# arnauqb/GradABM-JUNE

Hardware: AMD Instinct MI355X
Metric: simulation steps/sec (higher is better)
Workload: dtype f32

## Files before the change

### gradabm-june_amd/csrc/gj_tiled.h

```cpp
#pragma once
#include <hip/hip_runtime.h>
#include <stdint.h>

#include <type_traits>

#include "../../include/gradjune_hip.h"
#include "gj_device.h"

namespace gj {

constexpr int kTileThreads = 1024;
constexpr int kTileWaves = kTileThreads / kWave;
constexpr int kMaxSliceAgents = 19840;
constexpr int kUnroll = 8;
#ifndef GJ_UNROLL_NARROW
#define GJ_UNROLL_NARROW 16
#endif
constexpr int kUnrollNarrow = GJ_UNROLL_NARROW;
#ifndef GJ_VENUE_UNROLL
#define GJ_VENUE_UNROLL 2
#endif
constexpr int kVenueUnroll = GJ_VENUE_UNROLL;
#ifndef GJ_VENUE_UNROLL_C
#define GJ_VENUE_UNROLL_C GJ_VENUE_UNROLL
// ... 418 lines not shown
  const float* v_pc;
  float* cum;
  int32_t stride;
  int32_t nk;
  float beta[GJ_MAX_NETS_PER_SET];
  int32_t table[GJ_MAX_NETS_PER_SET];
  int32_t age75[GJ_MAX_NETS_PER_SET];
  int32_t leisure;
  int32_t direct;
  uint32_t term_limit;
  int32_t _pad_b;
  const uint16_t* pv_blk;
  const int32_t* blk_r0;
  const float* x;
  int64_t n_x;
};

struct TileBArgs {
  TSetB sets[GJ_MAX_SETS];
  const int32_t* work;
  const float* tables;
  int32_t day_type;
  int32_t mode;
  int32_t transpose;
  int32_t _pad;
};

struct ClassWeights {
  float l, lw;
};
__device__ __forceinline__ ClassWeights class_weights(const float* tables, int table, int age75, int day_type, int c) {
// ... 183 lines not shown
#pragma unroll
    for (int u = 0; u < kVenueUnroll; ++u) {
      const int gu = g + u * kTileThreads;
      if (gu >= gb) continue;
      Group8 G(raw[u], make_uint2(0u, 0u), xa[u], xb[u]);
#pragma unroll
      for (int q = 0; q < 8; ++q) {
        const int a = gu * 8 + q;
        if (!(a >= r0 && a < r1)) G.drop(q);
      }
      run_sums(W, G, 0, sums, vflags);
    }
  }
}

__device__ __forceinline__ void venue_cum_write(const VenueItem& W, const fx_t* sums, const uint32_t* vflags, float* cumf) {
  const TSetB& T = W.T;
  for (int l0 = W.tid; l0 < W.nv; l0 += kCumBatch * kTileThreads) {
    float pc[kCumBatch];
#pragma unroll
    for (int u = 0; u < kCumBatch; ++u) pc[u] = T.v_pc[W.v0 + min(l0 + u * kTileThreads, W.nv - 1)];
    for (int k = 0; k < W.nk; ++k) {
      const float beta = T.beta[k];
#pragma unroll
      for (int u = 0; u < kCumBatch; ++u) {
        const int lv = l0 + u * kTileThreads;
        if (lv < W.nv) {
          const float c = (beta * pc[u]) * fx_read<kFxVenue>(sums, vflags, W.vwords, k * W.nv + lv);
          T.cum[(int64_t)(W.v0 + lv) * T.stride + k] = c;
          cumf[2 * (k * W.nv + lv)] = c;
// ... 59 lines not shown
      store_nt(W.val4() + 2 * gu + 1, make_float4(r[4], r[5], r[6], r[7]));
    }
  }
}

#ifndef GJ_VENUE_WAVES_PER_SIMD
#define GJ_VENUE_WAVES_PER_SIMD 4
#endif
__global__ __launch_bounds__(kTileThreads, GJ_VENUE_WAVES_PER_SIMD) void k_tile_venues(const TileBArgs B) {
  extern __shared__ __align__(16) float lds_s[];
  [[maybe_unused]] const VenueStamp gj_stamp;
  const int set = B.work[2 * blockIdx.x], j = B.work[2 * blockIdx.x + 1];
  const TSetB& T = B.sets[set];
  if (T.nk == 0) return;
  const VenueItem W(T, j, lds_s, threadIdx.x);
  if (T.leisure) fill_class_weights<true, true>(W.tabs, W.tabs + W.nk * 200, T, B.tables, B.day_type, B.transpose, W.tid);
  if (B.mode != 2) {
    venue_zero(W, W.sums, W.vflags);
    __syncthreads();
    venue_sums_tiled(W, W.tabs, W.sums, W.vflags);
    if (T.pv_blk) venue_sums_runs(W, j, W.sums, W.vflags);
    __syncthreads();
    venue_cum_write(W, W.sums, W.vflags, W.cumf);
    if (B.mode == 1 || T.direct) return;
  } else {
    if (T.direct) return;
    venue_cum_read(W, W.cumf);
  }
  __syncthreads();
  venue_gather(W, W.tabs + W.nk * 200, W.cumf);
}

constexpr int GJ_MAX_PRESUM = 6;
constexpr int64_t kPresumBad = (int64_t)0x8000000000000000ll;
struct TPSet {
  const uint16_t* ell;
  int64_t plane_stride;
  fx_t* partial;
  int32_t planes, V, stride, nk;
  int32_t group_venues;
  int32_t raw, leisure, _pad;
  int32_t table[GJ_MAX_NETS_PER_SET];
  int32_t age75[GJ_MAX_NETS_PER_SET];
};
struct TilePArgs {
  TPSet sets[GJ_MAX_PRESUM];
  int32_t n_sets;
  int32_t agents_per_wg;
  int64_t n_agents;
  const float* trans;
  const float* qtrans;
  const uint8_t* cls;
  const float* tables;
  int32_t day_type, transpose;
};

constexpr int kPresumQuads = 3;
__device__ __forceinline__ void fx_add_or_poison(fx_t* sums, uint32_t* flags, int i, float x) {
  const bool ok = fabsf(x) <= fx_max<kFxVenue>();
  atomicAdd(&sums[i], to_fx<kFxVenue>(ok ? x : 0.0f));
  if (__builtin_expect(!ok, 0)) atomicOr(&flags[i >> 5], 1u << (i & 31));
}

__global__ __launch_bounds__(kTileThreads) void k_tile_presum(const TilePArgs P) {
  extern __shared__ __align__(16) fx_t lds_p[];
  const int tid = threadIdx.x;
  const int64_t a_begin = (int64_t)blockIdx.x * P.agents_per_wg;
  const int64_t a_end = min(P.n_agents, a_begin + P.agents_per_wg);
  const int n_quads = (int)((max(a_end - a_begin, (int64_t)0) + 3) >> 2);
  for (int t = 0; t < P.n_sets; ++t) {
    const TPSet& T = P.sets[t];
    const int nk = T.nk;
    const float* x = T.raw ? P.trans : P.qtrans;
    for (int v0 = 0; v0 < T.V; v0 += T.group_venues) {
      const int nv = min(T.group_venues, T.V - v0);
      const int n_sums = nv * nk;
      const int dummy = n_sums + (tid & 63);
      float* wtab = reinterpret_cast<float*>(lds_p + n_sums + 64);
      uint32_t* flags = reinterpret_cast<uint32_t*>(wtab + (T.leisure ? nk * 200 : 0));
      __syncthreads();
      for (int i = tid; i < n_sums + 64; i += kTileThreads) lds_p[i] = 0;
      for (int i = tid; i < (n_sums + 64 + 31) / 32; i += kTileThreads) flags[i] = 0u;
      if (T.leisure) fill_class_weights<true, false>(wtab, nullptr, T, P.tables, P.day_type, P.transpose, tid);
      __syncthreads();
      for (int plane = 0; plane < T.planes; ++plane) {
        const uint16_t* ell = T.ell + plane * T.plane_stride + a_begin * 2;
        struct Batch {
          uint4 rows[kPresumQuads];
          float4 xs[kPresumQuads];
          uint32_t cl[kPresumQuads];
        };
        auto load = [&](int b0, Batch& B) {
#pragma unroll
          for (int u = 0; u < kPresumQuads; ++u) {
            const int q = min(b0 + tid + u * kTileThreads, n_quads - 1);
            const int64_t a0 = a_begin + 4 * (int64_t)q;
            B.rows[u] = *reinterpret_cast<const uint4*>(ell + 8 * (int64_t)q);
            if (a0 + 4 <= P.n_agents) {
              B.xs[u] = *reinterpret_cast<const float4*>(x + a0);
            } else {
              B.xs[u] = make_float4(a0 < P.n_agents ? x[a0] : 0.0f, a0 + 1 < P.n_agents ? x[a0 + 1] : 0.0f,
                                    a0 + 2 < P.n_agents ? x[a0 + 2] : 0.0f, 0.0f);
            }
            B.cl[u] = T.leisure ? *reinterpret_cast<const uint32_t*>(P.cls + a0) : 0u;
          }
        };
        auto add = [&](int b0, const Batch& B) {
#pragma unroll
          for (int u = 0; u < kPresumQuads; ++u) {
            const int q = b0 + tid + u * kTileThreads;
            if (q >= n_quads) continue;
            const uint32_t w[4] = {B.rows[u].x, B.rows[u].y, B.rows[u].z, B.rows[u].w};
            const float xv[4] = {B.xs[u].x, B.xs[u].y, B.xs[u].z, B.xs[u].w};
            const int n_ok = (int)min((int64_t)4, a_end - (a_begin + 4 * (int64_t)q));
#pragma unroll
            for (int j = 0; j < 4; ++j) {
#pragma unroll
              for (int c = 0; c < 2; ++c) {
                const int lv = (int)((w[j] >> (16 * c)) & 0xFFFF) - v0;
                const bool in = ((unsigned)lv < (unsigned)nv) && (j < n_ok);
                if (!T.leisure) {
                  fx_add_or_poison(lds_p, flags, in ? lv : dummy, in ? xv[j] : 0.0f);
                } else {
                  const int cj = class_byte(B.cl[u], j);
                  for (int k = 0; k < nk; ++k)
                    fx_add_or_poison(lds_p, flags, in ? lv * nk + k : dummy, in ? wtab[k * 200 + cj] * xv[j] : 0.0f);
                }
              }
            }
          }
        };
        constexpr int kStep = kPresumQuads * kTileThreads;
        if (n_quads > 0) {
          Batch ba, bb;
          int b0 = 0;
          load(b0, ba);
          while (true) {
            const bool more1 = b0 + kStep < n_quads;
            if (more1) load(b0 + kStep, bb);
            add(b0, ba);
            if (!more1) break;
            b0 += kStep;
            const bool more2 = b0 + kStep < n_quads;
            if (more2) load(b0 + kStep, ba);
            add(b0, bb);
            if (!more2) break;
            b0 += kStep;
          }
        }
      }
      __syncthreads();
      fx_t* out = T.partial + (int64_t)blockIdx.x * T.V * T.stride;
      for (int i = tid; i < n_sums; i += kTileThreads) {
        const int lv = i / nk, k = i % nk;
        const bool bad = (flags[i >> 5] >> (i & 31)) & 1u;
        out[(int64_t)(v0 + lv) * T.stride + k] = bad ? (fx_t)kPresumBad : lds_p[i];
      }
    }
  }
}

struct PReduceSet {
  const fx_t* partial;
  const float* v_pc;
  float* cum;
  int32_t V, stride, nk, first;
  float beta[GJ_MAX_NETS_PER_SET];
};
struct PReduceArgs {
  PReduceSet sets[GJ_MAX_PRESUM];
  int32_t n_sets, n_wgs;
  int32_t total;
  int32_t _pad;
};

__global__ __launch_bounds__(kThreads) void k_presum_reduce(const PReduceArgs R) {
  __shared__ fx_t part[kThreads / kWave][kWave];
  __shared__ uint32_t bad_any[kWave];
  const int lane = threadIdx.x % kWave, wave = threadIdx.x / kWave;
  const int i = blockIdx.x * kWave + lane;
  const bool in = i < R.total;
  int t = 0;
  while (t + 1 < R.n_sets && i >= R.sets[t + 1].first) ++t;
  const PReduceSet& T = R.sets[t];
  const int e = in ? i - T.first : 0;
  const int v = e / T.nk, k = e % T.nk;
  const int64_t idx = (int64_t)v * T.stride + k, table = (int64_t)T.V * T.stride;
  fx_t s = 0;
  bool bad = false;
  if (threadIdx.x < kWave) bad_any[threadIdx.x] = 0u;
  constexpr int kWaves = kThreads / kWave;
  for (int w0 = wave; w0 < R.n_wgs; w0 += kWaves * 8) {
    fx_t p[8];
#pragma unroll
    for (int u = 0; u < 8; ++u) {
      const int w = w0 + u * kWaves;
      p[u] = (in && w < R.n_wgs) ? T.partial[w * table + idx] : (fx_t)0;
    }
#pragma unroll
    for (int u = 0; u < 8; ++u) {
      bad |= p[u] == (fx_t)kPresumBad;
      s += p[u];
    }
  }
  part[wave][lane] = s;
  __syncthreads();
  if (bad) atomicOr(&bad_any[lane], 1u);
  __syncthreads();
  if (wave == 0 && in) {
    fx_t total = 0;
#pragma unroll
    for (int w = 0; w < kWaves; ++w) total += part[w][lane];
    T.cum[idx] = (T.beta[k] * T.v_pc[v]) * (bad_any[lane] ? __builtin_nanf("") : from_fx<kFxVenue>(total));
  }
}

constexpr int GJ_MAX_DIRECT = GJ_MAX_SETS;
constexpr int kClassWeightFloats = GJ_MAX_NETS_PER_SET * 200;
struct TDirect {
  const uint16_t* ell;
  const float* cum;
  int64_t plane_stride;
  int32_t planes;
  int32_t V, stride, nk;
  int32_t region;
  int32_t group_venues;
  int32_t raw, leisure;
  int32_t table[GJ_MAX_NETS_PER_SET];
// ... 518 lines not shown
```

### gradabm-june_amd/csrc/gradjune_hip.hip

```cpp
#include <hip/hip_runtime.h>
#include <math.h>
#include <stdint.h>
#include <string.h>

#include "../../include/gradjune_hip.h"
#include "gj_device.h"
#include "gj_tiled.h"
#include "gj_agent.h"
#include "gj_location.h"

namespace gj {

struct SetP1 {
  const int32_t* v_rowptr;
  const int32_t* v_agent;
  const float* v_pc;
  float* cum;
  int32_t stride;
  int32_t nk;
  float beta[GJ_MAX_NETS_PER_SET];
  int32_t table[GJ_MAX_NETS_PER_SET];
  int32_t raw;
  int32_t leisure;
};
// ... 719 lines not shown
    sets[s].presum = uses_presum(plan, s);
    sets[s].raw = group_is_raw(p, G, g);
    sets[s].wide = S.desc_wide;
    sets[s].direct = S.ell_k != 0;
    sets[s].multi_slots = S.multi_slots;
  }
}

static size_t slice_lds(const gj_tiled* T, size_t elem) { return (size_t)T->slice_agents * elem; }
static size_t agents_lds(const gj_tiled* T) { return (size_t)T->slice_agents * sizeof(fx_t) + 2 * ((size_t)T->slice_agents / 8); }

static inline bool classes_by_dword(const gj_plan* plan) {
  return plan->agent_class && (uintptr_t)plan->agent_class % 4 == 0;
}

static int presum_fill(const gj_plan* plan, const gj_step_params* p, const Groups& G, int g, TPSet* X) {
  const gj_tiled* T = plan->tiled;
  const int s = G.set[g];
  const gj_tiled_set& S = T->sets[s];
  const gj_edge_set& E = plan->sets[s];
  const int64_t owned_slices = (plan->n_agents + T->slice_agents - 1) / T->slice_agents;
  X->ell = S.ell;
  X->plane_stride = owned_slices * (int64_t)T->slice_agents * 2;
  X->partial = reinterpret_cast<fx_t*>(S.presum);
  X->planes = S.ell_k / 2;
  X->V = (int32_t)E.n_venues;
  X->stride = E.cum_stride;
  const NetGroup C = classify_group(p, G, g);
  X->nk = C.nk;
  X->raw = C.raw;
  X->leisure = C.leisure;
  X->_pad = 0;
  memcpy(X->table, C.table, sizeof(X->table));
  memcpy(X->age75, C.age75, sizeof(X->age75));
  if (C.leisure && !classes_by_dword(plan)) return GJ_E_PLAN;
  return check_group(C);
}

static int tiled_presum(const gj_plan* plan, const gj_agent_state* st, const gj_step_params* p, const Groups& G,
                        hipStream_t stream) {
  const gj_tiled* T = plan->tiled;
  TilePArgs P;
  P.n_sets = 0;
  for (int g = 0; g < G.n; ++g) {
    if (!uses_presum(plan, G.set[g])) continue;
    if (P.n_sets == GJ_MAX_PRESUM) return GJ_E_PLAN;
    const int rc = presum_fill(plan, p, G, g, &P.sets[P.n_sets++]);
    if (rc) return rc;
  }
  if (P.n_sets == 0 || plan->n_agents == 0) return GJ_OK;
  const int64_t budget = 160 * 1024;
  size_t lds = 0;
  for (int t = 0; t < P.n_sets; ++t) {
    TPSet& X = P.sets[t];
    const int64_t fixed = 64 * 8 + (X.leisure ? (int64_t)X.nk * 200 * 4 : 0) + 64;
    int64_t per_venue = (int64_t)X.nk * 8;
    int64_t gv = (budget - fixed) * 8 / (per_venue * 8 + X.nk);
    if (T->direct_table_floats > 0 && gv > T->direct_table_floats / X.nk) gv = T->direct_table_floats / X.nk;
    if (gv > X.V) gv = X.V;
    if (gv < 1) gv = 1;
    X.group_venues = (int32_t)gv;
    const size_t need = (size_t)(gv * X.nk + 64) * 8 + (X.leisure ? (size_t)X.nk * 200 * 4 : 0) + ((size_t)(gv * X.nk + 64 + 31) / 32) * 4;
    if (need > lds) lds = need;
  }
  int64_t apw = (plan->n_agents + T->presum_wgs - 1) / T->presum_wgs;
  apw = (apw + 63) / 64 * 64;
  P.agents_per_wg = (int32_t)apw;
  P.n_agents = plan->n_agents;
  P.trans = st->transmission;
  P.qtrans = p->has_quarantine ? st->q_transmission : st->transmission;
  if (!aligned16(P.trans, P.qtrans)) return GJ_E_PLAN;
  P.cls = plan->agent_class;
  P.tables = plan->tables;
  P.day_type = p->day_type;
  P.transpose = p->transpose;
  int rc = allow_lds(k_tile_presum, lds);
  if (rc) return rc;
  return launch(k_tile_presum, T->presum_wgs, kTileThreads, lds, stream, P);
}

static int tiled_presum_reduce(const gj_plan* plan, const gj_step_params* p, const Groups& G, hipStream_t stream) {
  const gj_tiled* T = plan->tiled;
  PReduceArgs R;
  R.n_sets = 0;
  R.n_wgs = T->presum_wgs;
  R._pad = 0;
  int64_t total = 0;
  for (int g = 0; g < G.n; ++g) {
    const int s = G.set[g];
    if (!uses_presum(plan, s)) continue;
    if (R.n_sets == GJ_MAX_PRESUM) return GJ_E_PLAN;
    PReduceSet& X = R.sets[R.n_sets++];
    const gj_edge_set& E = plan->sets[s];
    X.partial = reinterpret_cast<const fx_t*>(T->sets[s].presum);
    X.v_pc = E.v_pcontact;
    X.cum = E.cum;
    X.V = (int32_t)E.n_venues;
    X.stride = E.cum_stride;
    X.nk = G.nk[g];
    X.first = (int32_t)total;
    const NetGroup C = classify_group(p, G, g);
    memcpy(X.beta, C.beta, sizeof(X.beta));
    total += (int64_t)X.V * X.nk;
  }
  if (R.n_sets == 0 || total == 0) return GJ_OK;
  if (total > INT32_MAX) return GJ_E_RANGE;
  R.total = (int32_t)total;
  return launch(k_presum_reduce, grid_for(total, 0, kWave), kThreads, 0, stream, R);
}

static int tiled_scatter(const gj_plan* plan, const gj_agent_state* st, const gj_step_params* p, const Groups& G,
                         hipStream_t stream) {
  const gj_tiled* T = plan->tiled;
  if (plan->n_ext_agents == 0 || G.n == 0) return GJ_OK;
  TileAArgs A;
  fill_set_a(plan, p, G, A.sets);
  A.n_sets = plan->n_sets;
  A.slice_agents = T->slice_agents;
  A.n_agents = plan->n_ext_agents;
  A.trans = st->transmission;
  A.qtrans = p->has_quarantine ? st->q_transmission : st->transmission;
  const size_t lds = slice_lds(T, sizeof(float));
  int rc = allow_lds(k_tile_scatter, lds);
  if (rc) return rc;
  rc = launch(k_tile_scatter, T->n_slices, kTileThreads, lds, stream, A);
  if (rc) return rc;
  return tiled_presum(plan, st, p, G, stream);
}

static uint32_t venue_term_limit(int32_t max_venue_edges) {
  int e = 14;
  int64_t p2 = 4096;
  while (p2 < (int64_t)max_venue_edges && e > -20) {
    p2 <<= 1;
    --e;
  }
  const float lim = ldexpf(1.0f, e);
  uint32_t bits;
  memcpy(&bits, &lim, sizeof(bits));
  return bits;
}

static int tiled_venues(const gj_plan* plan, const gj_agent_state* st, const gj_step_params* p, const Groups& G, int mode,
                        hipStream_t stream) {
  const gj_tiled* T = plan->tiled;
  if (G.n == 0) return GJ_OK;
  if (T->n_work == 0) return mode == 2 ? GJ_OK : tiled_presum_reduce(plan, p, G, stream);
  TileBArgs B;
  for (int s = 0; s < GJ_MAX_SETS; ++s) B.sets[s] = TSetB{};
  size_t lds = 16;
  for (int g = 0; g < G.n; ++g) {
    const int s = G.set[g];
    const gj_tiled_set& S = T->sets[s];
    const gj_edge_set& E = plan->sets[s];
    TSetB& X = B.sets[s];
    X.blk_v0 = S.blk_v0;
    X.blk_e0 = S.blk_e0;
    X.e_lv = S.e_lv;
    X.e_cls = S.e_cls;
    X.val = S.val;
    X.v_pc = E.v_pcontact;
    X.cum = E.cum;
    X.stride = E.cum_stride;
    X.nk = S.n_blocks > 0 ? G.nk[g] : 0;
    if (uses_presum(plan, s)) X.nk = 0;
    X.direct = S.ell_k != 0;
    const NetGroup C = classify_group(p, G, g);
    X.leisure = C.leisure;
    memcpy(X.beta, C.beta, sizeof(X.beta));
    memcpy(X.table, C.table, sizeof(X.table));
    memcpy(X.age75, C.age75, sizeof(X.age75));
    if (C.leisure && !S.e_cls && E.n_edges > 0) return GJ_E_PLAN;
    if (const int rc = check_group(C)) return rc;
    X.pv_blk = nullptr;
    X.blk_r0 = nullptr;
    X.x = nullptr;
    X.n_x = 0;
    if (S.run_pv_blk && mode != 2) {
      if (X.leisure) return GJ_E_PLAN;
      X.x = (p->has_quarantine && !C.raw) ? st->q_transmission : st->transmission;
// ... 4 lines not shown
      X.n_x = plan->n_ext_agents;
    }
    const size_t n_sums = (size_t)X.nk * S.max_block_venues + 64;
    const size_t need = n_sums * sizeof(fx_t) + (X.leisure ? 2 * 200 * (size_t)X.nk : 0) * sizeof(float) +
                        2 * ((n_sums + 31) / 32 * 4);
    X.term_limit = venue_term_limit(S.max_venue_edges);
    if (X.nk && need > lds) lds = need;
  }
  B.work = T->work;
  B.tables = plan->tables;
  B.day_type = p->day_type;
  B.mode = mode;
  B.transpose = p->transpose;
  int rc = allow_lds(k_tile_venues, lds);
  if (rc) return rc;
  rc = launch(k_tile_venues, T->n_work, kTileThreads, lds, stream, B);
  if (rc || mode == 2) return rc;
  return tiled_presum_reduce(plan, p, G, stream);
}

static int tiled_agents(const gj_plan* plan, const gj_agent_state* st, const gj_step_params* p, const Groups& G,
                        const gj_step_io* io, int sample, hipStream_t stream) {
  const gj_tiled* T = plan->tiled;
  if (plan->n_agents == 0) return GJ_OK;
  TileDArgs D;
  fill_set_a(plan, p, G, D.sets);
  D.n_sets = plan->n_sets;
  D.slice_agents = T->slice_agents;
  D.n_agents = plan->n_agents;
  D.stage = st->current_stage;
  D.susceptibility = st->susceptibility;
  D.is_infected = st->is_infected;
  D.infection_time = st->infection_time;
// ... 789 lines not shown
```

### gradabm-june_amd/grad_june_amd/plan.py

```python
from __future__ import annotations

import os

import ctypes as C
from dataclasses import dataclass, field
from typing import Dict, List, Optional, Sequence

import numpy as np
import torch

from . import _native as N
from . import tiling as TL

LONG_CHUNK = 8192
MAX_ROWS_PER_BLOCK = 2048


@dataclass
class HostEdgeSet:
    name: str
    n_venues: int
    n_edges: int
    v_rowptr: Optional[np.ndarray]
    v_agent: Optional[np.ndarray]
# ... 160 lines not shown
            if getattr(s, k) is not None:
                out[p + k] = getattr(s, k)
        if s.tiled is not None:
            t = s.tiled
            for k in ("blk_v0", "blk_e0", "e_lv", "e_cls", "a_la", "tile_sptr", "tile_jpos", "chunk_ptr", "chunk_desc", "ell",
                      "slot_idx", "multi_slots"):
                if getattr(t, k) is not None:
                    a = _host(getattr(t, k))
                    out[p + "tiled/" + k] = a.view(np.uint16) if (k in ("e_lv", "a_la", "ell") and a.dtype == np.int16) else a
            if t.runs is not None:
                for k in ("vmin", "pv_blk", "pv_win", "blk_r0", "win_lo", "win_n"):
                    a = _host(getattr(t.runs, k))
                    out[p + "tiled/runs/" + k] = a.view(np.uint16) if a.dtype == np.int16 else a
                out[p + "tiled/runs/meta"] = np.array([t.runs.n_primary, t.runs.max_window], dtype=np.int64)
            out[p + "tiled/meta"] = np.array([t.n_slices, t.n_blocks, t.n_slots, int(t.desc_wide), int(t.ell_k),
                                              int(t.presum)], dtype=np.int64)
    np.savez(path, **out)


def load_plan(path) -> HostPlan:
    with np.load(path, allow_pickle=False) as z:
        a = {k: z[k] for k in z.files}
    sets = []
    for name in str(a["meta/sets"]).split(","):
        if not name:
            continue
        p = f"set/{name}/"
        hs = HostEdgeSet(name, int(a[p + "n_venues"]), int(a[p + "n_edges"]), a.get(p + "v_rowptr"), a.get(p + "v_agent"),
                         a[p + "v_pcontact"], a.get(p + "a_rowptr"), a.get(p + "a_venue"))
        if p + "max_edges" in a:
            hs.max_venue_edges, hs.max_agent_edges = (int(x) for x in a[p + "max_edges"])
        if p + "tiled/meta" in a:
            meta = [int(x) for x in a[p + "tiled/meta"]]
            S, J, n_slots, wide = meta[:4]
            ell_k = meta[4] if len(meta) > 4 else 0
            hs.tiled = TL.TiledEdgeSet(name=name, n_venues=hs.n_venues, n_edges=hs.n_edges, n_slices=S, n_blocks=J,
                                       blk_v0=a[p + "tiled/blk_v0"], blk_e0=a[p + "tiled/blk_e0"], e_lv=a[p + "tiled/e_lv"],
                                       e_cls=a.get(p + "tiled/e_cls"), a_la=a[p + "tiled/a_la"],
                                       tile_sptr=a[p + "tiled/tile_sptr"], tile_jpos=a[p + "tiled/tile_jpos"],
                                       v_pcontact=hs.v_pcontact, n_slots=n_slots, chunk_ptr=a[p + "tiled/chunk_ptr"],
                                       chunk_desc=a[p + "tiled/chunk_desc"], desc_wide=bool(wide),
                                       ell=a.get(p + "tiled/ell"), ell_k=ell_k, slot_idx=a.get(p + "tiled/slot_idx"),
                                       multi_slots=a.get(p + "tiled/multi_slots"),
                                       presum=bool(meta[5]) if len(meta) > 5 else False)
            if p + "tiled/runs/meta" in a:
                r = p + "tiled/runs/"
                hs.tiled.n_edges = int(len(a[p + "tiled/a_la"]))
                hs.tiled.runs = TL.RunForm(n_primary=int(a[r + "meta"][0]), keep=None, vmin=a[r + "vmin"],
                                           pv_blk=a[r + "pv_blk"], pv_win=a[r + "pv_win"], blk_r0=a[r + "blk_r0"],
                                           win_lo=a[r + "win_lo"], win_n=a[r + "win_n"], max_window=int(a[r + "meta"][1]))
        sets.append(hs)
    return HostPlan(int(a["meta/n_agents"]), int(a["meta/n_ext_agents"]), sets, a["agent_class"], a["blocks"],
                    a["long_rows"], int(a["meta/n_partial_slots"]), {s.name: i for i, s in enumerate(sets)},
                    layout=str(a["meta/layout"]), n_slices=int(a["meta/n_slices"]),
                    slice_agents=int(a["meta/slice_agents"]), work=a.get("work"))


def agent_class_of(age, sex) -> np.ndarray:
    age = np.asarray(age).astype(np.int64)
# ... 10 lines not shown
                 nets_per_set: Optional[Dict[str, int]] = None, progress=None,
                 desc_wide: Optional[bool] = None, device=None, direct=None, runs=None, presum=None,
                 desc_explicit: Optional[bool] = None, multi_net_block_div: Optional[int] = None) -> HostPlan:
    if len(edge_sets) > N.GJ_MAX_SETS:
        raise ValueError(f"at most {N.GJ_MAX_SETS} edge sets")
    if layout not in ("csr", "tiled", "both"):
        raise ValueError(layout)
    n_ext = n_agents if n_ext_agents is None else n_ext_agents
    want_csr, want_tiled = layout in ("csr", "both"), layout in ("tiled", "both")
    cls_all = None if age is None else agent_class_of(age, sex)
    S, SA = slices if slices is not None else TL.choose_slices(n_ext)
    if eb_target is None:
        eb_target = TL.choose_block_edges(S)
    if multi_net_block_div is None:
        multi_net_block_div = int(os.environ.get("GJ_MULTI_NET_BLOCK_DIV", "1"))
    if want_tiled and n_ext != n_agents and (-(-n_agents // SA)) * SA > n_ext:
        raise ValueError("halo agents must start on a slice boundary (pad the owned range to a multiple of SA)")
    sets, all_blocks, all_long, work = [], [], [], []
    slot = 0
    n_presum = 0
    for sid, (name, es) in enumerate(edge_sets.items()):
        if device is not None and not want_csr:
            hs = _edge_set_on_device(name, es, n_ext, n_agents)
        else:
            hs = compile_edge_set(name, _host(es["agent"]), _host(es["venue"]), _host(es["people"]), n_agents, n_ext,
                                  csr=want_csr)
        sets.append(hs)
        if want_tiled:
            k = (nets_per_set or {}).get(name, 6 if name in leisure_sets else 1)
            use_cls = cls_all if (name in leisure_sets and cls_all is not None) else None
            forced_run = runs is not None and runs is not False and name in runs
            plan_direct = None
            if not forced_run:
                plan_direct = _direct_plan(name, es, hs.n_venues, n_agents, SA, k, direct, device)
            rf, es_t = None, es
# ... 8 lines not shown

                hs.tiled = build_tiled_native(name, es_t["agent"], es_t["venue"], hs.n_venues, hs.v_pcontact, S, SA,
                                              agent_class=use_cls, sv_max=max(16, sv_max // max(1, k)),
                                              eb_target=eb_set, wide=desc_wide, device=device, n_ext_agents=n_ext,
                                              explicit=desc_explicit)
            else:
                hs.tiled = TL.build_tiled(name, es_t["agent"], es_t["venue"], hs.n_venues, hs.v_pcontact, S, SA,
                                          agent_class=use_cls, sv_max=max(16, sv_max // max(1, k)),
                                          eb_target=eb_set, wide=desc_wide, explicit=desc_explicit,
                                          tile_pad=tile_pad)
            t = hs.tiled
            if rf is not None:
                t.runs = _finish_runs(rf, t, n_agents, SA, device)
            elif plan_direct is not None:
                t.ell, t.ell_k = plan_direct()
                t.presum = presum is True and plan_direct.all_owned and n_presum < 6
                n_presum += int(t.presum)
            blk_e0, blk_v0 = _host(t.blk_e0).astype(np.int64), _host(t.blk_v0).astype(np.int64)
            prim = np.diff(_host(t.runs.blk_r0).astype(np.int64)) if t.runs is not None else np.zeros(t.n_blocks, np.int64)
            for j in range(t.n_blocks):
                work.append((int(blk_e0[j + 1] - blk_e0[j]) + int(blk_v0[j + 1] - blk_v0[j]) + int(prim[j]), sid, j))
        if progress:
            progress(f"compiled edge set {name}")
        if not want_csr:
            continue
        b, lr, ns = build_schedule(hs.v_rowptr, sid, slot)
        slot += ns
        all_blocks.append(b)
        all_long.append(lr)
    blocks = np.concatenate(all_blocks) if all_blocks else np.zeros((0, 8), np.int32)
    long_rows = np.concatenate(all_long) if all_long else np.zeros((0, 4), np.int32)
    if block_order == "interleave" and len(blocks):
        order = np.argsort(-(blocks[:, 5] - blocks[:, 4]), kind="stable")
        blocks = blocks[order]
    if age is None:
        cls = np.zeros(n_ext, dtype=np.uint8)
# ... 108 lines not shown
        tabs = []
        for n in networks:
            if n.table is not None:
                self.table_index[n.name] = len(tabs)
                tabs.append(np.asarray(n.table, dtype=np.float32).reshape(N.GJ_TABLE_SIZE))
        self.tables = up(np.stack(tabs)) if tabs else None

        per_set_nets: Dict[str, int] = {}
        for n in networks:
            if n.edge_set not in host.set_index:
                raise KeyError(f"network {n.name}: edge set {n.edge_set!r} not in the world")
            per_set_nets[n.edge_set] = per_set_nets.get(n.edge_set, 0) + 1
        self.keep = []
        self.cum: List[torch.Tensor] = []
        self.tiled_c = None
        by_name = {s.name: s for s in host.sets}
        flat_sizes = {n: max(1, by_name[n].n_venues) * max(1, per_set_nets.get(n, 1))
                      for n in flat_cum_sets if n in by_name}
        self.flat_cum = (torch.zeros(sum(flat_sizes.values()), dtype=torch.float32, device=dev)
                         if flat_sizes else None)
        self.flat_offsets: Dict[str, tuple] = {}
        off = 0
        for n, size in flat_sizes.items():
            self.flat_offsets[n] = (off, size)
            off += size
        plan = N.Plan()
        plan.n_agents = host.n_agents
        plan.n_ext_agents = host.n_ext_agents
        plan.n_sets = len(host.sets)
        for i, s in enumerate(host.sets):
# ... 69 lines not shown
        plan.n_blocks = len(host.blocks)
        plan.n_long_rows = len(host.long_rows)
        plan.n_partial_slots = host.n_partial_slots
        plan.blocks = N.ptr(self.blocks)
        plan.long_rows = N.ptr(self.long_rows)
        plan.partial = N.ptr(self.partial)
        plan.agent_class = N.ptr(self.agent_class)
        plan.tables = N.ptr(self.tables)
        plan.n_tables = len(tabs)
        if self.tiled_c is not None:
            self.work = up(host.work.reshape(-1)) if len(host.work) else None
            self.tiled_c.n_work = len(host.work)
            self.tiled_c.work = N.ptr(self.work)
            self.agent_scratch = (torch.zeros(max(1, host.n_agents), dtype=torch.float32, device=dev)
                                  if split_epilogue else None)
            wgs = int(min(256, max(1, -(-host.n_agents // 4096))))
            for i, s_ in enumerate(host.sets):
                if s_.tiled is not None and s_.tiled.presum and s_.tiled.ell_k:
                    stride = int(plan.sets[i].cum_stride)
                    buf = torch.zeros(wgs * max(1, s_.n_venues) * stride, dtype=torch.int64, device=dev)
                    self.keep[i]["presum"] = buf
                    self.tiled_c.sets[i].presum = buf.data_ptr()
                    self.tiled_c.presum_wgs = wgs
            self.tiled_c.agent_scratch = N.ptr(self.agent_scratch)
            plan.tiled = C.pointer(self.tiled_c)
        self.c = plan

    def cum_of(self, set_name: str) -> torch.Tensor:
        i = self.host.set_index[set_name]
        stride = self.c.sets[i].cum_stride
        return self.cum[i][: self.host.sets[i].n_venues * stride].view(self.host.sets[i].n_venues, stride)

    def location_rows(self, edges=None):
        if getattr(self, "_location_rows", None) is not None:
            return self._location_rows
# ... 40 lines not shown
```

### gradabm-june_amd/grad_june_amd/tiling.py

```python
from __future__ import annotations

from dataclasses import dataclass
from typing import Optional

import numpy as np

SA_MAX = 19840
MAX_AGENT_EDGES = 4096
SV_MAX = 16384
EB_TARGET = 131072
N_CU = 256
PAD = 8
CHUNK = 64


def choose_slices(n_agents: int, sa_max: int = SA_MAX, n_cu: int = N_CU):
    if n_agents <= 0:
        return 1, 64
    if n_agents <= n_cu * 1024:
        sa = 1024 if n_agents > 1024 * 8 else max(64, -(-n_agents // 8))
        sa = -(-sa // 64) * 64
        s = -(-n_agents // sa)
        return s, sa
    m = -(-n_agents // (n_cu * sa_max))
# ... 38 lines not shown
    e_cls: Optional[np.ndarray]
    a_la: np.ndarray
    tile_sptr: np.ndarray
    tile_jpos: np.ndarray
    v_pcontact: np.ndarray
    n_slots: int = 0
    chunk_ptr: Optional[np.ndarray] = None
    chunk_desc: Optional[np.ndarray] = None
    desc_wide: bool = False
    slot_idx: Optional[np.ndarray] = None
    multi_slots: Optional[np.ndarray] = None
    ell: Optional[np.ndarray] = None
    ell_k: int = 0
    runs: Optional["RunForm"] = None
    presum: bool = False


WIDE_SEGMENTS = 6
WIDE_MIN_SHARE = 0.05
EXPLICIT_MIN_SHARE = 0.02


def wide_descriptors(sptr: np.ndarray, jpos_flat: np.ndarray, seg: np.ndarray, chunk_ptr: np.ndarray,
                     first_edge: np.ndarray, chunk_end: np.ndarray, t0: np.ndarray, J: int):
    n_chunks = len(first_edge)
    E = int(sptr[-1])
    tile_len = np.diff(sptr)
    starts_all = sptr[:-1][tile_len > 0]
    tile_ids = np.flatnonzero(tile_len > 0)
    lo = np.searchsorted(starts_all, first_edge, side="right")
# ... 250 lines not shown
    k = 2
    while k < degree_max:
        k *= 2
    return k


def direct_eligible(n_venues: int, n_edges_owned: int, n_agents: int, degree_max: int, nets: int,
                    slice_agents: int) -> bool:
    if n_edges_owned == 0 or n_venues > DIRECT_MAX_VENUES or degree_max > DIRECT_MAX_K:
        return False
    if n_venues * max(1, nets) > DIRECT_TABLE_GROUPS * direct_table_floats(slice_agents):
        return False
    return direct_columns(degree_max) * n_agents <= DIRECT_MAX_PAD * n_edges_owned


def ell_planes(ell_rows_by_k, K: int):
    if K <= 2:
        return ell_rows_by_k.reshape(1, ell_rows_by_k.shape[0], K)
    rows = ell_rows_by_k.shape[0]
    return ell_rows_by_k.reshape(rows, K // 2, 2).transpose(1, 0, 2) if isinstance(ell_rows_by_k, np.ndarray) \
        else ell_rows_by_k.reshape(rows, K // 2, 2).permute(1, 0, 2)


def build_ell(agent_index, venue_index, n_agents: int, n_slices_owned: int, slice_agents: int):
    agent = np.asarray(agent_index, dtype=np.int64).ravel()
    venue = np.asarray(venue_index, dtype=np.int64).ravel()
    owned = agent < n_agents
    a, v = agent[owned], venue[owned]
    order = np.argsort(a, kind="stable")
    a, v = a[order], v[order]
# ... 98 lines not shown
```

Measured before the change: 2056.

## Fold presum partial reduction into venue kernel and auto-select presum sets

```diff
diff --git a/gradabm-june_amd/csrc/gj_tiled.h b/gradabm-june_amd/csrc/gj_tiled.h
--- a/gradabm-june_amd/csrc/gj_tiled.h
+++ b/gradabm-june_amd/csrc/gj_tiled.h
@@ -456,7 +456,12 @@
   const int32_t* blk_r0;
   const float* x;
   int64_t n_x;
-};
+  const fx_t* presum;
+  int32_t presum_wgs;
+  int32_t presum_entries;
+};
+__host__ __device__ constexpr int64_t presum_flag_words(int64_t n) { return 2 * ((n + 63) / 64); }
+__host__ __device__ constexpr int64_t presum_table_units(int64_t n) { return n + presum_flag_words(n); }
 
 struct TileBArgs {
   TSetB sets[GJ_MAX_SETS];
@@ -670,6 +675,57 @@
   }
 }
 
+constexpr int kPresumTables = 8;
+__device__ __forceinline__ void venue_sums_presum(const VenueItem& W, fx_t* sums, uint32_t* vflags) {
+  const TSetB& T = W.T;
+  const int stride = T.stride, n_e = W.nv * stride, n_wgs = T.presum_wgs;
+  const int64_t unit = presum_table_units(T.presum_entries);
+  {
+    const fx_t* base = T.presum + (int64_t)W.v0 * stride;
+    const int span = min(n_e, kTileThreads), G = kTileThreads / span, tg = W.tid / span;
+    if (tg < G) {
+      for (int e = W.tid - tg * span; e < n_e; e += span) {
+        fx_t s = 0;
+        for (int w0 = tg; w0 < n_wgs; w0 += kPresumTables * G) {
+          fx_t p[kPresumTables];
+#pragma unroll
+          for (int u = 0; u < kPresumTables; ++u)
+            p[u] = __builtin_nontemporal_load(base + (int64_t)min(w0 + u * G, n_wgs - 1) * unit + e);
+#pragma unroll
+          for (int u = 0; u < kPresumTables; ++u) s += (w0 + u * G < n_wgs) ? p[u] : (fx_t)0;
+        }
+        const int lv = e / stride, k = e % stride;
+        if (k < W.nk) atomicAdd(&sums[k * W.nv + lv], s);
+      }
+    }
+  }
+  const int g_lo = W.v0 * stride, w_lo = g_lo >> 5, nw = ((g_lo + n_e - 1) >> 5) - w_lo + 1;
+  const int fwords = (int)presum_flag_words(T.presum_entries);
+  const uint32_t* fbase = reinterpret_cast<const uint32_t*>(T.presum + T.presum_entries);
+  const int span = min(2 * nw, kTileThreads), G = kTileThreads / span, tg = W.tid / span;
+  if (tg < G) {
+    for (int j = W.tid - tg * span; j < 2 * nw; j += span) {
+      const int neg = j >= nw, wi = w_lo + j - neg * nw;
+      const uint32_t* f = fbase + neg * fwords + wi;
+      uint32_t m = 0u;
+      for (int w0 = tg; w0 < n_wgs; w0 += kPresumTables * G) {
+        uint32_t p[kPresumTables];
+#pragma unroll
+        for (int u = 0; u < kPresumTables; ++u) p[u] = f[(int64_t)min(w0 + u * G, n_wgs - 1) * unit * 2];
+#pragma unroll
+        for (int u = 0; u < kPresumTables; ++u) m |= (w0 + u * G < n_wgs) ? p[u] : 0u;
+      }
+      while (m) {
+        const int g = wi * 32 + __builtin_ctz(m) - g_lo;
+        m &= m - 1u;
+        if ((unsigned)g >= (unsigned)n_e || g % stride >= W.nk) continue;
+        const int i = (g % stride) * W.nv + g / stride;
+        atomicOr(&vflags[neg * W.vwords + (i >> 5)], 1u << (i & 31));
+      }
+    }
+  }
+}
+
 __device__ __forceinline__ void venue_cum_write(const VenueItem& W, const fx_t* sums, const uint32_t* vflags, float* cumf) {
   const TSetB& T = W.T;
   for (int l0 = W.tid; l0 < W.nv; l0 += kCumBatch * kTileThreads) {
@@ -759,12 +815,16 @@
   const TSetB& T = B.sets[set];
   if (T.nk == 0) return;
   const VenueItem W(T, j, lds_s, threadIdx.x);
-  if (T.leisure) fill_class_weights<true, true>(W.tabs, W.tabs + W.nk * 200, T, B.tables, B.day_type, B.transpose, W.tid);
+  if (T.leisure && !T.presum) fill_class_weights<true, true>(W.tabs, W.tabs + W.nk * 200, T, B.tables, B.day_type, B.transpose, W.tid);
   if (B.mode != 2) {
     venue_zero(W, W.sums, W.vflags);
     __syncthreads();
-    venue_sums_tiled(W, W.tabs, W.sums, W.vflags);
-    if (T.pv_blk) venue_sums_runs(W, j, W.sums, W.vflags);
+    if (T.presum) {
+      venue_sums_presum(W, W.sums, W.vflags);
+    } else {
+      venue_sums_tiled(W, W.tabs, W.sums, W.vflags);
+      if (T.pv_blk) venue_sums_runs(W, j, W.sums, W.vflags);
+    }
     __syncthreads();
     venue_cum_write(W, W.sums, W.vflags, W.cumf);
     if (B.mode == 1 || T.direct) return;
@@ -777,14 +837,14 @@
 }
 
 constexpr int GJ_MAX_PRESUM = 6;
-constexpr int64_t kPresumBad = (int64_t)0x8000000000000000ll;
 struct TPSet {
   const uint16_t* ell;
   int64_t plane_stride;
   fx_t* partial;
   int32_t planes, V, stride, nk;
   int32_t group_venues;
-  int32_t raw, leisure, _pad;
+  int32_t raw, leisure;
+  uint32_t term_limit;
   int32_t table[GJ_MAX_NETS_PER_SET];
   int32_t age75[GJ_MAX_NETS_PER_SET];
 };
@@ -801,10 +861,12 @@
 };
 
 constexpr int kPresumQuads = 3;
-__device__ __forceinline__ void fx_add_or_poison(fx_t* sums, uint32_t* flags, int i, float x) {
-  const bool ok = fabsf(x) <= fx_max<kFxVenue>();
-  atomicAdd(&sums[i], to_fx<kFxVenue>(ok ? x : 0.0f));
-  if (__builtin_expect(!ok, 0)) atomicOr(&flags[i >> 5], 1u << (i & 31));
+__device__ __forceinline__ void presum_term(fx_t* sums, uint32_t* flags, int words, uint32_t limit, int i, float x) {
+  if (__builtin_expect(abs_bits(x) <= limit, 1)) {
+    atomicAdd(&sums[i], to_fx<kFxVenue>(x));
+  } else {
+    fx_flag(flags, words, i, x);
+  }
 }
 
 __global__ __launch_bounds__(kTileThreads) void k_tile_presum(const TilePArgs P) {
@@ -816,41 +878,56 @@
   for (int t = 0; t < P.n_sets; ++t) {
     const TPSet& T = P.sets[t];
     const int nk = T.nk;
+    const uint32_t limit = T.term_limit;
     const float* x = T.raw ? P.trans : P.qtrans;
+    const int n_tot = T.V * T.stride;
+    fx_t* out = T.partial + (int64_t)blockIdx.x * presum_table_units(n_tot);
+    uint32_t* gflags = reinterpret_cast<uint32_t*>(out + n_tot);
+    const int gwords = (int)presum_flag_words(n_tot);
+    for (int i = tid; i < 2 * gwords; i += kTileThreads) gflags[i] = 0u;
     for (int v0 = 0; v0 < T.V; v0 += T.group_venues) {
       const int nv = min(T.group_venues, T.V - v0);
       const int n_sums = nv * nk;
-      const int dummy = n_sums + (tid & 63);
-      float* wtab = reinterpret_cast<float*>(lds_p + n_sums + 64);
+      const int words = (n_sums + 31) / 32;
+      float* wtab = reinterpret_cast<float*>(lds_p + n_sums);
       uint32_t* flags = reinterpret_cast<uint32_t*>(wtab + (T.leisure ? nk * 200 : 0));
+      struct Batch {
+        uint4 rows[kPresumQuads];
+        float4 xs[kPresumQuads];
+        uint32_t cl[kPresumQuads];
+      };
+      auto load = [&](int plane, int b0, Batch& B) {
+        const uint16_t* ell = T.ell + plane * T.plane_stride + a_begin * 2;
+#pragma unroll
+        for (int u = 0; u < kPresumQuads; ++u) {
+          const int q = min(b0 + tid + u * kTileThreads, n_quads - 1);
+          const int64_t a0 = a_begin + 4 * (int64_t)q;
+          B.rows[u] = *reinterpret_cast<const uint4*>(ell + 8 * (int64_t)q);
+          if (a0 + 4 <= P.n_agents) {
+            B.xs[u] = *reinterpret_cast<const float4*>(x + a0);
+          } else {
+            B.xs[u] = make_float4(a0 < P.n_agents ? x[a0] : 0.0f, a0 + 1 < P.n_agents ? x[a0 + 1] : 0.0f,
+                                  a0 + 2 < P.n_agents ? x[a0 + 2] : 0.0f, 0.0f);
+          }
+          B.cl[u] = T.leisure ? *reinterpret_cast<const uint32_t*>(P.cls + a0) : 0u;
+        }
+      };
+      Batch ba, bb;
+      if (n_quads > 0) load(0, 0, ba);
       __syncthreads();
-      for (int i = tid; i < n_sums + 64; i += kTileThreads) lds_p[i] = 0;
-      for (int i = tid; i < (n_sums + 64 + 31) / 32; i += kTileThreads) flags[i] = 0u;
+      for (int i = tid; i < n_sums; i += kTileThreads) lds_p[i] = 0;
+      for (int i = tid; i < 2 * words; i += kTileThreads) flags[i] = 0u;
       if (T.leisure) fill_class_weights<true, false>(wtab, nullptr, T, P.tables, P.day_type, P.transpose, tid);
       __syncthreads();
       for (int plane = 0; plane < T.planes; ++plane) {
-        const uint16_t* ell = T.ell + plane * T.plane_stride + a_begin * 2;
-        struct Batch {
-          uint4 rows[kPresumQuads];
-          float4 xs[kPresumQuads];
-          uint32_t cl[kPresumQuads];
-        };
-        auto load = [&](int b0, Batch& B) {
+        auto add = [&](int b0, const Batch& B) {
+          bool some = false;
 #pragma unroll
           for (int u = 0; u < kPresumQuads; ++u) {
-            const int q = min(b0 + tid + u * kTileThreads, n_quads - 1);
-            const int64_t a0 = a_begin + 4 * (int64_t)q;
-            B.rows[u] = *reinterpret_cast<const uint4*>(ell + 8 * (int64_t)q);
-            if (a0 + 4 <= P.n_agents) {
-              B.xs[u] = *reinterpret_cast<const float4*>(x + a0);
-            } else {
-              B.xs[u] = make_float4(a0 < P.n_agents ? x[a0] : 0.0f, a0 + 1 < P.n_agents ? x[a0 + 1] : 0.0f,
-                                    a0 + 2 < P.n_agents ? x[a0 + 2] : 0.0f, 0.0f);
-            }
-            B.cl[u] = T.leisure ? *reinterpret_cast<const uint32_t*>(P.cls + a0) : 0u;
+            const bool live = b0 + tid + u * kTileThreads < n_quads;
+            some |= live && (B.xs[u].x != 0.0f || B.xs[u].y != 0.0f || B.xs[u].z != 0.0f || B.xs[u].w != 0.0f);
           }
-        };
-        auto add = [&](int b0, const Batch& B) {
+          if (__builtin_amdgcn_ballot_w64(some) == 0ull) return;
 #pragma unroll
           for (int u = 0; u < kPresumQuads; ++u) {
             const int q = b0 + tid + u * kTileThreads;
@@ -864,12 +941,13 @@
               for (int c = 0; c < 2; ++c) {
                 const int lv = (int)((w[j] >> (16 * c)) & 0xFFFF) - v0;
                 const bool in = ((unsigned)lv < (unsigned)nv) && (j < n_ok);
-                if (!T.leisure) {
-                  fx_add_or_poison(lds_p, flags, in ? lv : dummy, in ? xv[j] : 0.0f);
-                } else {
-                  const int cj = class_byte(B.cl[u], j);
-                  for (int k = 0; k < nk; ++k)
-                    fx_add_or_poison(lds_p, flags, in ? lv * nk + k : dummy, in ? wtab[k * 200 + cj] * xv[j] : 0.0f);
+                if (in && xv[j] != 0.0f) {
+                  if (!T.leisure) {
+                    presum_term(lds_p, flags, words, limit, lv, xv[j]);
+                  } else {
+                    const int cj = class_byte(B.cl[u], j);
+                    for (int k = 0; k < nk; ++k) presum_term(lds_p, flags, words, limit, lv * nk + k, wtab[k * 200 + cj] * xv[j]);
+                  }
                 }
               }
             }
@@ -877,17 +955,16 @@
         };
         constexpr int kStep = kPresumQuads * kTileThreads;
         if (n_quads > 0) {
-          Batch ba, bb;
           int b0 = 0;
-          load(b0, ba);
+          if (plane > 0) load(plane, b0, ba);
           while (true) {
             const bool more1 = b0 + kStep < n_quads;
-            if (more1) load(b0 + kStep, bb);
+            if (more1) load(plane, b0 + kStep, bb);
             add(b0, ba);
             if (!more1) break;
             b0 += kStep;
             const bool more2 = b0 + kStep < n_quads;
-            if (more2) load(b0 + kStep, ba);
+            if (more2) load(plane, b0 + kStep, ba);
             add(b0, bb);
             if (!more2) break;
             b0 += kStep;
@@ -895,68 +972,21 @@
         }
       }
       __syncthreads();
-      fx_t* out = T.partial + (int64_t)blockIdx.x * T.V * T.stride;
       for (int i = tid; i < n_sums; i += kTileThreads) {
         const int lv = i / nk, k = i % nk;
-        const bool bad = (flags[i >> 5] >> (i & 31)) & 1u;
-        out[(int64_t)(v0 + lv) * T.stride + k] = bad ? (fx_t)kPresumBad : lds_p[i];
-      }
-    }
-  }
-}
-
-struct PReduceSet {
-  const fx_t* partial;
-  const float* v_pc;
-  float* cum;
-  int32_t V, stride, nk, first;
-  float beta[GJ_MAX_NETS_PER_SET];
-};
-struct PReduceArgs {
-  PReduceSet sets[GJ_MAX_PRESUM];
-  int32_t n_sets, n_wgs;
-  int32_t total;
-  int32_t _pad;
-};
-
-__global__ __launch_bounds__(kThreads) void k_presum_reduce(const PReduceArgs R) {
-  __shared__ fx_t part[kThreads / kWave][kWave];
-  __shared__ uint32_t bad_any[kWave];
-  const int lane = threadIdx.x % kWave, wave = threadIdx.x / kWave;
-  const int i = blockIdx.x * kWave + lane;
-  const bool in = i < R.total;
-  int t = 0;
-  while (t + 1 < R.n_sets && i >= R.sets[t + 1].first) ++t;
-  const PReduceSet& T = R.sets[t];
-  const int e = in ? i - T.first : 0;
-  const int v = e / T.nk, k = e % T.nk;
-  const int64_t idx = (int64_t)v * T.stride + k, table = (int64_t)T.V * T.stride;
-  fx_t s = 0;
-  bool bad = false;
-  if (threadIdx.x < kWave) bad_any[threadIdx.x] = 0u;
-  constexpr int kWaves = kThreads / kWave;
-  for (int w0 = wave; w0 < R.n_wgs; w0 += kWaves * 8) {
-    fx_t p[8];
-#pragma unroll
-    for (int u = 0; u < 8; ++u) {
-      const int w = w0 + u * kWaves;
-      p[u] = (in && w < R.n_wgs) ? T.partial[w * table + idx] : (fx_t)0;
-    }
-#pragma unroll
-    for (int u = 0; u < 8; ++u) {
-      bad |= p[u] == (fx_t)kPresumBad;
-      s += p[u];
-    }
-  }
-  part[wave][lane] = s;
-  __syncthreads();
-  if (bad) atomicOr(&bad_any[lane], 1u);
-  __syncthreads();
-  if (wave == 0 && in) {
-    fx_t total = 0;
-#pragma unroll
-    for (int w = 0; w < kWaves; ++w) total += part[w][lane];
-    T.cum[idx] = (T.beta[k] * T.v_pc[v]) * (bad_any[lane] ? __builtin_nanf("") : from_fx<kFxVenue>(total));
+        out[(int64_t)(v0 + lv) * T.stride + k] = lds_p[i];
+      }
+      for (int w = tid; w < 2 * words; w += kTileThreads) {
+        uint32_t m = flags[w];
+        const int neg = w >= words;
+        while (m) {
+          const int i = (w - neg * words) * 32 + __builtin_ctz(m);
+          m &= m - 1u;
+          const int g = (v0 + i / nk) * T.stride + i % nk;
+          atomicOr(&gflags[neg * gwords + (g >> 5)], 1u << (g & 31));
+        }
+      }
+    }
   }
 }
 
diff --git a/gradabm-june_amd/csrc/gradjune_hip.hip b/gradabm-june_amd/csrc/gradjune_hip.hip
--- a/gradabm-june_amd/csrc/gradjune_hip.hip
+++ b/gradabm-june_amd/csrc/gradjune_hip.hip
@@ -757,6 +757,8 @@
   return plan->agent_class && (uintptr_t)plan->agent_class % 4 == 0;
 }
 
+static uint32_t venue_term_limit(int32_t max_venue_edges);
+
 static int presum_fill(const gj_plan* plan, const gj_step_params* p, const Groups& G, int g, TPSet* X) {
   const gj_tiled* T = plan->tiled;
   const int s = G.set[g];
@@ -773,7 +775,7 @@
   X->nk = C.nk;
   X->raw = C.raw;
   X->leisure = C.leisure;
-  X->_pad = 0;
+  X->term_limit = venue_term_limit(S.max_venue_edges);
   memcpy(X->table, C.table, sizeof(X->table));
   memcpy(X->age75, C.age75, sizeof(X->age75));
   if (C.leisure && !classes_by_dword(plan)) return GJ_E_PLAN;
@@ -793,17 +795,17 @@
   }
   if (P.n_sets == 0 || plan->n_agents == 0) return GJ_OK;
   const int64_t budget = 160 * 1024;
-  size_t lds = 0;
+  size_t lds = 16;
   for (int t = 0; t < P.n_sets; ++t) {
     TPSet& X = P.sets[t];
-    const int64_t fixed = 64 * 8 + (X.leisure ? (int64_t)X.nk * 200 * 4 : 0) + 64;
-    int64_t per_venue = (int64_t)X.nk * 8;
-    int64_t gv = (budget - fixed) * 8 / (per_venue * 8 + X.nk);
+    if ((int64_t)X.V * X.stride > INT32_MAX) return GJ_E_RANGE;
+    const int64_t fixed = (X.leisure ? (int64_t)X.nk * 200 * 4 : 0) + 16;
+    int64_t gv = (budget - fixed) * 4 / ((int64_t)X.nk * 33);
     if (T->direct_table_floats > 0 && gv > T->direct_table_floats / X.nk) gv = T->direct_table_floats / X.nk;
     if (gv > X.V) gv = X.V;
     if (gv < 1) gv = 1;
     X.group_venues = (int32_t)gv;
-    const size_t need = (size_t)(gv * X.nk + 64) * 8 + (X.leisure ? (size_t)X.nk * 200 * 4 : 0) + ((size_t)(gv * X.nk + 64 + 31) / 32) * 4;
+    const size_t need = (size_t)(gv * X.nk) * 8 + (X.leisure ? (size_t)X.nk * 200 * 4 : 0) + 2 * ((size_t)(gv * X.nk + 31) / 32) * 4;
     if (need > lds) lds = need;
   }
   int64_t apw = (plan->n_agents + T->presum_wgs - 1) / T->presum_wgs;
@@ -822,40 +824,12 @@
   return launch(k_tile_presum, T->presum_wgs, kTileThreads, lds, stream, P);
 }
 
-static int tiled_presum_reduce(const gj_plan* plan, const gj_step_params* p, const Groups& G, hipStream_t stream) {
-  const gj_tiled* T = plan->tiled;
-  PReduceArgs R;
-  R.n_sets = 0;
-  R.n_wgs = T->presum_wgs;
-  R._pad = 0;
-  int64_t total = 0;
-  for (int g = 0; g < G.n; ++g) {
-    const int s = G.set[g];
-    if (!uses_presum(plan, s)) continue;
-    if (R.n_sets == GJ_MAX_PRESUM) return GJ_E_PLAN;
-    PReduceSet& X = R.sets[R.n_sets++];
-    const gj_edge_set& E = plan->sets[s];
-    X.partial = reinterpret_cast<const fx_t*>(T->sets[s].presum);
-    X.v_pc = E.v_pcontact;
-    X.cum = E.cum;
-    X.V = (int32_t)E.n_venues;
-    X.stride = E.cum_stride;
-    X.nk = G.nk[g];
-    X.first = (int32_t)total;
-    const NetGroup C = classify_group(p, G, g);
-    memcpy(X.beta, C.beta, sizeof(X.beta));
-    total += (int64_t)X.V * X.nk;
-  }
-  if (R.n_sets == 0 || total == 0) return GJ_OK;
-  if (total > INT32_MAX) return GJ_E_RANGE;
-  R.total = (int32_t)total;
-  return launch(k_presum_reduce, grid_for(total, 0, kWave), kThreads, 0, stream, R);
-}
-
 static int tiled_scatter(const gj_plan* plan, const gj_agent_state* st, const gj_step_params* p, const Groups& G,
                          hipStream_t stream) {
   const gj_tiled* T = plan->tiled;
   if (plan->n_ext_agents == 0 || G.n == 0) return GJ_OK;
+  int rc = tiled_presum(plan, st, p, G, stream);
+  if (rc) return rc;
   TileAArgs A;
   fill_set_a(plan, p, G, A.sets);
   A.n_sets = plan->n_sets;
@@ -864,11 +838,9 @@
   A.trans = st->transmission;
   A.qtrans = p->has_quarantine ? st->q_transmission : st->transmission;
   const size_t lds = slice_lds(T, sizeof(float));
-  int rc = allow_lds(k_tile_scatter, lds);
-  if (rc) return rc;
-  rc = launch(k_tile_scatter, T->n_slices, kTileThreads, lds, stream, A);
-  if (rc) return rc;
-  return tiled_presum(plan, st, p, G, stream);
+  rc = allow_lds(k_tile_scatter, lds);
+  if (rc) return rc;
+  return launch(k_tile_scatter, T->n_slices, kTileThreads, lds, stream, A);
 }
 
 static uint32_t venue_term_limit(int32_t max_venue_edges) {
@@ -888,7 +860,7 @@
                         hipStream_t stream) {
   const gj_tiled* T = plan->tiled;
   if (G.n == 0) return GJ_OK;
-  if (T->n_work == 0) return mode == 2 ? GJ_OK : tiled_presum_reduce(plan, p, G, stream);
+  if (T->n_work == 0) return GJ_OK;
   TileBArgs B;
   for (int s = 0; s < GJ_MAX_SETS; ++s) B.sets[s] = TSetB{};
   size_t lds = 16;
@@ -906,7 +878,15 @@
     X.cum = E.cum;
     X.stride = E.cum_stride;
     X.nk = S.n_blocks > 0 ? G.nk[g] : 0;
-    if (uses_presum(plan, s)) X.nk = 0;
+    X.presum = nullptr;
+    X.presum_wgs = 0;
+    X.presum_entries = 0;
+    if (uses_presum(plan, s)) {
+      if ((int64_t)E.n_venues * E.cum_stride > INT32_MAX) return GJ_E_RANGE;
+      X.presum = reinterpret_cast<const fx_t*>(S.presum);
+      X.presum_wgs = T->presum_wgs;
+      X.presum_entries = (int32_t)(E.n_venues * E.cum_stride);
+    }
     X.direct = S.ell_k != 0;
     const NetGroup C = classify_group(p, G, g);
     X.leisure = C.leisure;
@@ -941,9 +921,7 @@
   B.transpose = p->transpose;
   int rc = allow_lds(k_tile_venues, lds);
   if (rc) return rc;
-  rc = launch(k_tile_venues, T->n_work, kTileThreads, lds, stream, B);
-  if (rc || mode == 2) return rc;
-  return tiled_presum_reduce(plan, p, G, stream);
+  return launch(k_tile_venues, T->n_work, kTileThreads, lds, stream, B);
 }
 
 static int tiled_agents(const gj_plan* plan, const gj_agent_state* st, const gj_step_params* p, const Groups& G,
diff --git a/gradabm-june_amd/grad_june_amd/plan.py b/gradabm-june_amd/grad_june_amd/plan.py
--- a/gradabm-june_amd/grad_june_amd/plan.py
+++ b/gradabm-june_amd/grad_june_amd/plan.py
@@ -198,7 +198,7 @@
                     out[p + "tiled/runs/" + k] = a.view(np.uint16) if a.dtype == np.int16 else a
                 out[p + "tiled/runs/meta"] = np.array([t.runs.n_primary, t.runs.max_window], dtype=np.int64)
             out[p + "tiled/meta"] = np.array([t.n_slices, t.n_blocks, t.n_slots, int(t.desc_wide), int(t.ell_k),
-                                              int(t.presum)], dtype=np.int64)
+                                              int(t.presum), int(t.presum_auto)], dtype=np.int64)
     np.savez(path, **out)
 
 
@@ -226,7 +226,8 @@
                                        chunk_desc=a[p + "tiled/chunk_desc"], desc_wide=bool(wide),
                                        ell=a.get(p + "tiled/ell"), ell_k=ell_k, slot_idx=a.get(p + "tiled/slot_idx"),
                                        multi_slots=a.get(p + "tiled/multi_slots"),
-                                       presum=bool(meta[5]) if len(meta) > 5 else False)
+                                       presum=bool(meta[5]) if len(meta) > 5 else False,
+                                       presum_auto=bool(meta[6]) if len(meta) > 6 else False)
             if p + "tiled/runs/meta" in a:
                 r = p + "tiled/runs/"
                 hs.tiled.n_edges = int(len(a[p + "tiled/a_la"]))
@@ -267,11 +268,13 @@
         eb_target = TL.choose_block_edges(S)
     if multi_net_block_div is None:
         multi_net_block_div = int(os.environ.get("GJ_MULTI_NET_BLOCK_DIV", "1"))
+    if presum is None and os.environ.get("GJ_PRESUM", "") in ("off", "on", "auto"):
+        presum = {"off": False, "on": True, "auto": "auto"}[os.environ["GJ_PRESUM"]]
     if want_tiled and n_ext != n_agents and (-(-n_agents // SA)) * SA > n_ext:
         raise ValueError("halo agents must start on a slice boundary (pad the owned range to a multiple of SA)")
     sets, all_blocks, all_long, work = [], [], [], []
     slot = 0
-    n_presum = 0
+    n_presum, presum_bytes = 0, 0
     for sid, (name, es) in enumerate(edge_sets.items()):
         if device is not None and not want_csr:
             hs = _edge_set_on_device(name, es, n_ext, n_agents)
@@ -310,12 +313,24 @@
                 t.runs = _finish_runs(rf, t, n_agents, SA, device)
             elif plan_direct is not None:
                 t.ell, t.ell_k = plan_direct()
-                t.presum = presum is True and plan_direct.all_owned and n_presum < 6
+                if presum is True:
+                    t.presum = plan_direct.all_owned and n_presum < TL.PRESUM_MAX_SETS
+                elif presum == "auto":
+                    k_min = k if name in (nets_per_set or {}) else 1
+                    tb = TL.presum_table_bytes(hs.n_venues, k_min, n_agents)
+                    t.presum = t.presum_auto = (
+                        TL.presum_eligible(hs.n_venues, hs.n_edges, hs.n_edges if plan_direct.all_owned else -1, n_agents,
+                                           n_ext, t.ell_k, k_min, leisure=use_cls is not None, nets_max=k)
+                        and n_presum < TL.PRESUM_MAX_SETS and presum_bytes + tb <= TL.PRESUM_CAP_BYTES)
+                    presum_bytes += tb if t.presum else 0
                 n_presum += int(t.presum)
             blk_e0, blk_v0 = _host(t.blk_e0).astype(np.int64), _host(t.blk_v0).astype(np.int64)
             prim = np.diff(_host(t.runs.blk_r0).astype(np.int64)) if t.runs is not None else np.zeros(t.n_blocks, np.int64)
+            table_slots = TL.presum_workgroups(n_agents) * k * 8 // 6 if t.presum else 0
             for j in range(t.n_blocks):
-                work.append((int(blk_e0[j + 1] - blk_e0[j]) + int(blk_v0[j + 1] - blk_v0[j]) + int(prim[j]), sid, j))
+                nv_j = int(blk_v0[j + 1] - blk_v0[j])
+                slots = nv_j * table_slots if t.presum else int(blk_e0[j + 1] - blk_e0[j])
+                work.append((slots + nv_j + int(prim[j]), sid, j))
         if progress:
             progress(f"compiled edge set {name}")
         if not want_csr:
@@ -454,6 +469,7 @@
         self.keep = []
         self.cum: List[torch.Tensor] = []
         self.tiled_c = None
+        self.presum_sets: List[str] = []
         by_name = {s.name: s for s in host.sets}
         flat_sizes = {n: max(1, by_name[n].n_venues) * max(1, per_set_nets.get(n, 1))
                       for n in flat_cum_sets if n in by_name}
@@ -553,11 +569,20 @@
             self.tiled_c.work = N.ptr(self.work)
             self.agent_scratch = (torch.zeros(max(1, host.n_agents), dtype=torch.float32, device=dev)
                                   if split_epilogue else None)
-            wgs = int(min(256, max(1, -(-host.n_agents // 4096))))
+            wgs = TL.presum_workgroups(host.n_agents)
+            presum_bytes = 0
             for i, s_ in enumerate(host.sets):
                 if s_.tiled is not None and s_.tiled.presum and s_.tiled.ell_k:
                     stride = int(plan.sets[i].cum_stride)
-                    buf = torch.zeros(wgs * max(1, s_.n_venues) * stride, dtype=torch.int64, device=dev)
+                    tb = TL.presum_table_bytes(s_.n_venues, stride, host.n_agents)
+                    if s_.tiled.presum_auto and not (
+                            TL.presum_eligible(s_.n_venues, s_.n_edges, s_.n_edges, host.n_agents, host.n_ext_agents,
+                                               s_.tiled.ell_k, stride, leisure=s_.tiled.e_cls is not None)
+                            and presum_bytes + tb <= TL.PRESUM_CAP_BYTES):
+                        continue
+                    presum_bytes += tb
+                    self.presum_sets.append(s_.name)
+                    buf = torch.zeros(tb // 8, dtype=torch.int64, device=dev)
                     self.keep[i]["presum"] = buf
                     self.tiled_c.sets[i].presum = buf.data_ptr()
                     self.tiled_c.presum_wgs = wgs
diff --git a/gradabm-june_amd/grad_june_amd/tiling.py b/gradabm-june_amd/grad_june_amd/tiling.py
--- a/gradabm-june_amd/grad_june_amd/tiling.py
+++ b/gradabm-june_amd/grad_june_amd/tiling.py
@@ -76,6 +76,7 @@
     ell_k: int = 0
     runs: Optional["RunForm"] = None
     presum: bool = False
+    presum_auto: bool = False
 
 
 WIDE_SEGMENTS = 6
@@ -356,6 +357,47 @@
     return direct_columns(degree_max) * n_agents <= DIRECT_MAX_PAD * n_edges_owned
 
 
+PRESUM_MAX_SETS = 6
+PRESUM_MAX_WGS = 256
+PRESUM_CAP_BYTES = 64 << 20
+PHASE_AB_BYTES_PER_EDGE = 12.3
+PRESUM_BYTES_FACTOR = 0.5
+
+
+def presum_workgroups(n_agents: int) -> int:
+    return int(min(PRESUM_MAX_WGS, max(1, -(-int(n_agents) // 1024))))
+
+
+def presum_table_bytes(n_venues: int, nets: int, n_agents: int) -> int:
+    n = max(1, int(n_venues)) * max(1, int(nets))
+    return presum_workgroups(n_agents) * (n + 2 * ((n + 63) // 64)) * 8
+
+
+def presum_lds_bytes(n_venues: int, nets: int, leisure: bool) -> int:
+    n = int(n_venues) * max(1, int(nets))
+    return n * 8 + (max(1, int(nets)) * 200 * 4 if leisure else 0) + 2 * ((n + 31) // 32) * 4
+
+
+def presum_eligible(n_venues: int, n_edges: int, n_edges_owned: int, n_agents: int, n_ext_agents: int, ell_k: int,
+                    nets: int, leisure: bool = False, nets_max: Optional[int] = None) -> bool:
+    if ell_k <= 0 or n_edges <= 0 or n_edges_owned != n_edges or n_ext_agents != n_agents:
+        return False
+    if presum_lds_bytes(n_venues, max(nets, nets_max or 0), leisure) > LDS_BYTES:
+        return False
+    rows = 2 * int(ell_k) * int(n_agents) + (int(n_agents) if leisure else 0)
+    return rows + 2 * presum_table_bytes(n_venues, nets, n_agents) <= PRESUM_BYTES_FACTOR * PHASE_AB_BYTES_PER_EDGE * n_edges
+
+
+def presum_choose(candidates, n_agents: int):
+    chosen, total = [], 0
+    for key, n_venues, nets in candidates:
+        b = presum_table_bytes(n_venues, nets, n_agents)
+        if len(chosen) < PRESUM_MAX_SETS and total + b <= PRESUM_CAP_BYTES:
+            chosen.append(key)
+            total += b
+    return chosen
+
+
 def ell_planes(ell_rows_by_k, K: int):
     if K <= 2:
         return ell_rows_by_k.reshape(1, ell_rows_by_k.shape[0], K)
```

Result: slower. 2027 (-1.4%).
